# vsergeev/luaradio

Hardware: NVIDIA H100
Metric: WBFM-mono chain Msamples/s (input samples) @N H100; FIR-128 HBM GB/s vs roofline (higher is better)
Workload: dtype f32

## Files before the change

luaradio_b200/csrc/tuner.cu:

```cuda
#include "common.cuh"
#include "blocks.h"

#include <cuda.h>
#include <cudaTypedefs.h>

#include <climits>
#include <cmath>
#include <cstdlib>
#include <cstring>
#include <new>
#include <string>
#include <type_traits>
#include <vector>

namespace lrb {

namespace {

#ifndef LRB_PT_THREADS
#define LRB_PT_THREADS 64
#define LRB_PT_R 8
#define LRB_PT_CTAS 8
#define LRB_PT_PREFETCH 9
#define LRB_PT_BATCH 7
#endif
#ifndef LRB_PT_EXPERIMENT
#define LRB_PT_EXPERIMENT 0
#endif
#ifndef LRB_PT_EARLY_REST
#define LRB_PT_EARLY_REST 0
#endif
constexpr int PT_THREADS = LRB_PT_THREADS;
constexpr int PT_R = LRB_PT_R;
constexpr int PT_TO = PT_THREADS * PT_R;
constexpr int PT_MAXTAPS = 144;
constexpr int PT_BATCH = LRB_PT_BATCH;

constexpr int PT_MAXIT = 48;
struct PolyParams {
    float hr[PT_MAXTAPS];
    float hs[PT_MAXTAPS / 2];
    float2 step[PT_MAXIT];
    uint64_t turns_fix;
    uint64_t g0;
    long long off;
    int M;
    float pole_c;
    float pole_cp[6];
};
constexpr int PT_POLE_WARM = (64 % LRB_PT_R == 0) ? 64 : ((72 % LRB_PT_R == 0) ? 72 : 4 * LRB_PT_R);
static_assert(PT_POLE_WARM % LRB_PT_R == 0 && PT_POLE_WARM % 4 == 0 && PT_POLE_WARM >= 64, "pole warm-up must cover whole threads");

template <int D, int Q>
struct PolyShape {
    static constexpr int RD = PT_R * D;
    static constexpr int T = Q * D + 1;
    static constexpr int SPAN = (PT_TO + Q - 1) * D + 1;
    static constexpr int PAIRS = (SPAN + 1) / 2;
    static constexpr int ITERS = (PAIRS + PT_THREADS - 1) / PT_THREADS;
    static constexpr int LOADED = 2 * ITERS * PT_THREADS;
    __host__ __device__ static constexpr int pad(int e) { return e + 2 * (e / RD); }
    static constexpr int ELEMS = LOADED + 2 * (LOADED / RD) + 2;
    static constexpr size_t SMEM = (size_t)ELEMS * sizeof(float2);
    static constexpr int ROWS = (SPAN + RD - 1) / RD;
    static constexpr int STAGED = ROWS * RD + 2;
    static constexpr size_t SMEM_BULK = (size_t)ROWS * (RD + 2) * sizeof(float2);
    static constexpr int PPS = RD / 2;
    static constexpr int RG = PT_THREADS / PPS;
    static constexpr int RITERS = (ROWS + RG - 1) / RG;
};

__device__ __forceinline__ uint32_t smem_addr(const void* p) { return (uint32_t)__cvta_generic_to_shared(p); }
__device__ __forceinline__ void mbar_init(uint64_t* bar) {
    asm volatile("mbarrier.init.shared::cta.b64 [%0], 1;\n\tfence.mbarrier_init.release.cluster;\n\t"
                 "fence.proxy.async.shared::cta;" :: "r"(smem_addr(bar)) : "memory");
}
__device__ __forceinline__ void mbar_expect_tx(uint64_t* bar, uint32_t bytes) {
    asm volatile("mbarrier.arrive.expect_tx.shared::cta.b64 _, [%0], %1;" :: "r"(smem_addr(bar)), "r"(bytes) : "memory");
}
__device__ __forceinline__ void mbar_wait(uint64_t* bar, uint32_t parity) {
    asm volatile("{\n\t.reg .pred p;\n\tLRB_WAIT_%=:\n\t"
                 "mbarrier.try_wait.parity.shared::cta.b64 p, [%0], %1;\n\t"
                 "@!p bra LRB_WAIT_%=;\n\t}" :: "r"(smem_addr(bar)), "r"(parity) : "memory");
}
__device__ __forceinline__ void fence_proxy_async() { asm volatile("fence.proxy.async.shared::cta;" ::: "memory"); }
__device__ __forceinline__ void tensor_g2s_2d(void* dst, const CUtensorMap* map, int c0, int c1, uint64_t* bar) {
    asm volatile("cp.async.bulk.tensor.2d.shared::cluster.global.tile.mbarrier::complete_tx::bytes [%0], [%1, {%2, %3}], [%4];"
                 :: "r"(smem_addr(dst)), "l"(reinterpret_cast<uint64_t>(map)), "r"(c0), "r"(c1), "r"(smem_addr(bar))
                 : "memory");
}

template <int B, int E, typename F>
__device__ __forceinline__ void static_for(F&& f) {
    if constexpr (B < E) {
        f(std::integral_constant<int, B>{});
        static_for<B + 1, E>(f);
    }
}

constexpr int DISC_OV = 4;
constexpr int DISC_TAIL = 4;
template <bool DISC>
struct TileStride { static constexpr int TS = DISC ? PT_TO - DISC_OV - DISC_TAIL : PT_TO; };

template <int D, int Q, bool ROT, bool DISC, bool EDGE, bool REAL = false, bool POLE = false>
__global__ void __launch_bounds__(PT_THREADS, LRB_PT_CTAS)
polyphase_crcf_kernel(const float2* __restrict__ x, const float2* __restrict__ hist, long long n,
                      void* __restrict__ yv, long long n_out, const __grid_constant__ PolyParams P,
                      const __grid_constant__ CUtensorMap tmap, long long t_lo, long long t_hi,
                      const float2* __restrict__ prev_in, float2* __restrict__ prev_out, float inv_gain) {
    using S = PolyShape<D, Q>;
    static_assert(!(REAL && (ROT || DISC)), "the real-stream variant has no translator / discriminator");
    static_assert(REAL || !POLE, "the fused pole exists in the real-stream variant only");
    constexpr int PW = POLE ? PT_POLE_WARM : 0;
    constexpr int PAY = PT_TO - PW;
    constexpr int TS = REAL ? 2 * PAY : TileStride<DISC>::TS;
    constexpr int NPRE = S::ITERS < LRB_PT_PREFETCH ? S::ITERS : LRB_PT_PREFETCH;
    constexpr int LANE1 = PAY * D;
    const float* __restrict__ xr = reinterpret_cast<const float*>(x);
    const float* __restrict__ histr = reinterpret_cast<const float*>(hist);
    extern __shared__ __align__(128) float2 smem[];
    __shared__ float2 s_edge[PT_THREADS / 32];
    const int tid = threadIdx.x, lane = tid & 31, warp = tid >> 5;
    const int Hm1 = P.M - 1;

    constexpr bool BULK = !EDGE && !REAL && DISC;
    constexpr bool FFA = BULK && LRB_PT_EXPERIMENT != 2;
    __shared__ float2 s_ffa[FFA ? 4 : 1][PT_THREADS / 32];
    __shared__ __align__(8) uint64_t s_bar;
    uint32_t bar_phase = 0;

    float2 A0 = make_float2(1.f, 0.f), A1 = make_float2(1.f, 0.f);
    const int rg = tid / S::PPS, rw = tid - rg * S::PPS;
    constexpr int NE0 = (BULK && ROT) ? S::RITERS : 1;
    float2 E0[NE0];
    float2 W1 = make_float2(1.f, 0.f);
    if constexpr (BULK && ROT) {
        W1 = phasor_from_fix(P.turns_fix);
#pragma unroll
        for (int it = 0; it < NE0; ++it)
            E0[it] = phasor_from_fix(P.turns_fix * (uint64_t)((rg + S::RG * it) * S::RD + 2 * rw));
    } else if constexpr (ROT) {
        A0 = phasor_from_fix(P.turns_fix * (uint64_t)(2 * tid));
        A1 = phasor_from_fix(P.turns_fix * (uint64_t)(2 * tid + 1));
    }
    const bool rot_last = rg < S::RG && rg + S::RG * (S::RITERS - 1) < S::ROWS;
    auto tile_of = [&](long long idx) -> long long { return EDGE ? (idx < t_lo ? idx : t_hi + (idx - t_lo)) : (t_lo + idx); };
    const long long n_work = EDGE ? 0 : (t_hi - t_lo);
    long long widx = blockIdx.x;

    constexpr int TILE_ROWS = TS * D / S::RD;
    static_assert(!BULK || (TS * D) % S::RD == 0, "tiles start on whole rows of the tensor map");
    auto issue_tile = [&](long long idx) {
        if (tid == 0) {
            fence_proxy_async();
            mbar_expect_tx(&s_bar, (uint32_t)S::SMEM_BULK);
            tensor_g2s_2d(smem, &tmap, 0, (int)(idx * TILE_ROWS), &s_bar);
        }
    };
    if constexpr (BULK) {
        if (tid == 0) mbar_init(&s_bar);
        __syncthreads();
        if (widx < n_work) issue_tile(widx);
    }

    auto ld_pair = [&](long long Bt, int k) -> float4 {
        if constexpr (REAL) {
            const float2* pa = reinterpret_cast<const float2*>(xr + Bt) + (tid + k * PT_THREADS);
            const float2 a = __ldcs(pa), b = __ldcs(pa + LANE1 / 2);
            return make_float4(a.x, b.x, a.y, b.y);
        } else {
            return __ldcs(reinterpret_cast<const float4*>(x + Bt) + (tid + k * PT_THREADS));
        }
    };
    float4 pre[NPRE];
    constexpr int REST = (S::ITERS - NPRE) < PT_BATCH ? (S::ITERS - NPRE) : PT_BATCH;
    float4 rest[REST > 0 ? REST : 1];
    if constexpr (!EDGE && !BULK) {
        if (widx < n_work) {
            const long long Bt = P.off + tile_of(widx) * (long long)(TS * D);
#pragma unroll
            for (int k = 0; k < NPRE; ++k) pre[k] = ld_pair(Bt, k);
            if constexpr (LRB_PT_EARLY_REST) {
#pragma unroll
                for (int k = 0; k < REST; ++k) rest[k] = ld_pair(Bt, NPRE + k);
            }
        }
    }

    for (;;) {
        if constexpr (!EDGE) { if (widx >= n_work) break; }
        const long long tile = tile_of(widx);
        const long long B = P.off + tile * (long long)(TS * D);
        const long long m0 = tile * TS - (DISC ? DISC_OV : 0) - PW;

        auto stage_pair = [&](float4 v, int it) {
            const int u = tid + it * PT_THREADS;
            float2 a = make_float2(v.x, v.y), b = make_float2(v.z, v.w);
            if constexpr (ROT) {
                const float2 st = P.step[it];
                a = cmul(a, cmul(A0, st));
                b = cmul(b, cmul(A1, st));
            }
            *reinterpret_cast<float4*>(smem + S::pad(2 * u)) = make_float4(a.x, a.y, b.x, b.y);
        };
        if constexpr (BULK) {
            if (LRB_PT_EXPERIMENT != 1 || widx == blockIdx.x) {
                if (LRB_PT_EXPERIMENT != 3 || widx == blockIdx.x) {
                    mbar_wait(&s_bar, bar_phase);
                    bar_phase ^= 1;
                }
                if (rg < S::RG) {
                    float2* row = smem + rg * (S::RD + 2) + 2 * rw;
#pragma unroll
                    for (int it = 0; it < S::RITERS; ++it) {
                        if (it == S::RITERS - 1 && !rot_last) break;
                        float4* p = reinterpret_cast<float4*>(row + it * S::RG * (S::RD + 2));
                        float4 v = *p;
                        if constexpr (ROT && LRB_PT_EXPERIMENT != 4) {
                            const float2 a = cmul(make_float2(v.x, v.y), E0[it]);
                            const float2 b = cmul(make_float2(v.z, v.w), cmul(E0[it], W1));
                            v = make_float4(a.x, a.y, b.x, b.y);
                        }
                        *p = v;
                    }
                }
            }
        } else if constexpr (!EDGE && LRB_PT_EXPERIMENT == 1) {
            if (widx == blockIdx.x) {
#pragma unroll 1
                for (int it = 0; it < S::ITERS; ++it) stage_pair(ld_pair(B, it), it);
            }
        } else if constexpr (!EDGE) {
            if constexpr (!LRB_PT_EARLY_REST) {
#pragma unroll
                for (int k = 0; k < REST; ++k) rest[k] = ld_pair(B, NPRE + k);
            }
#pragma unroll
            for (int k = 0; k < NPRE; ++k) stage_pair(pre[k], k);
#pragma unroll
            for (int k = 0; k < REST; ++k) stage_pair(rest[k], NPRE + k);
#pragma unroll 1
            for (int it0 = NPRE + REST; it0 < S::ITERS; it0 += PT_BATCH) {
                float4 buf[PT_BATCH];
#pragma unroll
                for (int k = 0; k < PT_BATCH; ++k)
                    if (it0 + k < S::ITERS) buf[k] = ld_pair(B, it0 + k);
#pragma unroll
                for (int k = 0; k < PT_BATCH; ++k)
                    if (it0 + k < S::ITERS) stage_pair(buf[k], it0 + k);
            }
        } else {
#pragma unroll 7
            for (int it = 0; it < S::ITERS; ++it) {
                const long long i0 = B + 2LL * (tid + it * PT_THREADS);
                if constexpr (REAL) {
                    auto g = [&](long long i) -> float {
                        return (i >= 0) ? (i < n ? __ldg(xr + i) : 0.f) : ((Hm1 + i >= 0) ? __ldg(histr + (Hm1 + i)) : 0.f);
                    };
                    stage_pair(make_float4(g(i0), g(i0 + LANE1), g(i0 + 1), g(i0 + 1 + LANE1)), it);
                    continue;
                }
                const float2 a = (i0 >= 0) ? (i0 < n ? __ldg(x + i0) : make_float2(0.f, 0.f))
                                           : ((Hm1 + i0 >= 0) ? __ldg(hist + (Hm1 + i0)) : make_float2(0.f, 0.f));
                const long long i1 = i0 + 1;
                const float2 b = (i1 >= 0) ? (i1 < n ? __ldg(x + i1) : make_float2(0.f, 0.f))
                                           : ((Hm1 + i1 >= 0) ? __ldg(hist + (Hm1 + i1)) : make_float2(0.f, 0.f));
                stage_pair(make_float4(a.x, a.y, b.x, b.y), it);
            }
        }
        __syncthreads();

        if constexpr (!EDGE && !BULK && LRB_PT_EXPERIMENT != 1) {
            const long long nidx = widx + gridDim.x;
            if (nidx < n_work) {
                const long long Bn = P.off + tile_of(nidx) * (long long)(TS * D);
#pragma unroll
                for (int k = 0; k < NPRE; ++k) pre[k] = ld_pair(Bn, k);
            }
        }

        float2 acc[PT_R];
#pragma unroll
        for (int r = 0; r < PT_R; ++r) acc[r] = make_float2(0.f, 0.f);
        const float2* tb = smem + tid * (S::RD + 2);
        auto load_block = [&](auto jc, float2 (&xs)[D]) {
            constexpr int j = decltype(jc)::value;
            constexpr int e0 = j * D;
            if constexpr (j == PT_R + Q - 1) {
                xs[0] = tb[S::pad(e0)];
            } else {
                static_for<0, D>([&](auto pc) {
                    constexpr int pp = decltype(pc)::value;
                    constexpr int e = e0 + pp;
                    if constexpr ((e & 1) && pp >= 1) {
                    } else if constexpr (!(e & 1) && pp + 1 < D) {
                        const float4 v = *reinterpret_cast<const float4*>(tb + S::pad(e));
                        xs[pp] = make_float2(v.x, v.y);
                        xs[pp + 1] = make_float2(v.z, v.w);
                    } else {
                        xs[pp] = tb[S::pad(e)];
                    }
                });
            }
        };
        float2 ffa_a0, ffa_fs, ffa_fb, ffa_sp;
        const float hq = P.hr[Q * D];
        if constexpr (FFA) {
            static_assert(Q % 2 == 0 && PT_R % 2 == 0 && (Q / 2) * D <= PT_MAXTAPS / 2, "fast-FIR split needs even Q and R");
            static_assert(DISC_TAIL >= 1, "the tile's last output has no A_{R/2}");
            constexpr int QH = Q / 2, KP = PT_R / 2;
            float2 fa[KP], fb[KP], fs[KP], uo[D], an;
#pragma unroll
            for (int k = 0; k < KP; ++k) fa[k] = fb[k] = fs[k] = make_float2(0.f, 0.f);
            static_for<0, PT_R + Q>([&](auto jc) {
                constexpr int j = decltype(jc)::value;
                float2 xs[D];
                load_block(jc, xs);
                if constexpr (j == PT_R + Q - 1) {
                } else if constexpr (j % 2 == 0) {
                    constexpr int i = j / 2;
                    static_for<0, KP>([&](auto kc) {
                        constexpr int k = decltype(kc)::value, q = i - k;
                        if constexpr (q >= 0 && q < QH) {
                            static_for<0, D>([&](auto pc) {
                                constexpr int pp = decltype(pc)::value;
                                const float h = P.hr[2 * q * D + pp];
                                fa[k] = ffma2(xs[pp], make_float2(h, h), fa[k]);
                            });
                        }
                    });
                    if constexpr (i >= 1 && i - 1 <= KP - 1 + QH - 1) {
                        float2 v[D];
#pragma unroll
                        for (int pp = 0; pp < D; ++pp) v[pp] = fadd2(uo[pp], xs[pp]);
                        static_for<0, KP>([&](auto kc) {
                            constexpr int k = decltype(kc)::value, q = i - 1 - k;
                            if constexpr (q >= 0 && q < QH) {
                                static_for<0, D>([&](auto pc) {
                                    constexpr int pp = decltype(pc)::value;
                                    const float h = P.hs[q * D + pp];
                                    fs[k] = ffma2(v[pp], make_float2(h, h), fs[k]);
                                });
                            }
                        });
                    }
                } else {
                    constexpr int i = (j - 1) / 2;
                    static_for<0, KP>([&](auto kc) {
                        constexpr int k = decltype(kc)::value, q = i - k;
                        if constexpr (q >= 0 && q < QH) {
                            static_for<0, D>([&](auto pc) {
                                constexpr int pp = decltype(pc)::value;
                                const float h = P.hr[(2 * q + 1) * D + pp];
                                fb[k] = ffma2(xs[pp], make_float2(h, h), fb[k]);
                            });
                        }
                    });
#pragma unroll
                    for (int pp = 0; pp < D; ++pp) uo[pp] = xs[pp];
                }
                if constexpr (j == 2 * QH - 1) {
                    an = make_float2(__shfl_down_sync(0xffffffffu, fa[0].x, 1), __shfl_down_sync(0xffffffffu, fa[0].y, 1));
                }
                if constexpr (j >= Q) {
                    constexpr int r = j - Q, k = r / 2;
                    if constexpr (r % 2 == 0) {
                        acc[r] = ffma2(xs[0], make_float2(hq, hq), fadd2(fa[k], fb[k]));
                    } else if constexpr (k + 1 < KP) {
                        acc[r] = ffma2(xs[0], make_float2(hq, hq), fsub2(fsub2(fs[k], fa[k + 1]), fb[k]));
                    } else {
                        acc[r] = ffma2(xs[0], make_float2(hq, hq), fsub2(fsub2(fs[k], an), fb[k]));
                        ffa_a0 = fa[0]; ffa_fs = fs[k]; ffa_fb = fb[k]; ffa_sp = xs[0];
                    }
                }
            });
        } else {
            static_for<0, (LRB_PT_EXPERIMENT == 2 ? 1 : PT_R + Q)>([&](auto jc) {
                constexpr int j = decltype(jc)::value;
                float2 xs[D];
                load_block(jc, xs);
                static_for<0, PT_R>([&](auto rc) {
                    constexpr int r = decltype(rc)::value;
                    constexpr int qq = j - r;
                    if constexpr (qq >= 0 && qq <= Q) {
                        static_for<0, D>([&](auto pc) {
                            constexpr int pp = decltype(pc)::value;
                            if constexpr (qq * D + pp < S::T) {
                                const float h = P.hr[qq * D + pp];
                                acc[r] = ffma2(xs[pp], make_float2(h, h), acc[r]);
                            }
                        });
                    }
                });
            });
        }
        if constexpr (!EDGE && !BULK && LRB_PT_EARLY_REST) {
            const long long nidx = widx + gridDim.x;
            if (nidx < n_work) {
                const long long Bn = P.off + tile_of(nidx) * (long long)(TS * D);
#pragma unroll
                for (int k = 0; k < REST; ++k) rest[k] = ld_pair(Bn, NPRE + k);
            }
        }
        if constexpr (ROT && !DISC) {
            const float2 Pt = phasor_from_fix(P.turns_fix * (P.g0 + (uint64_t)B));
#pragma unroll
            for (int r = 0; r < PT_R; ++r) acc[r] = cmul(acc[r], Pt);
        }

        const long long mbase = m0 + (long long)tid * PT_R;
        if constexpr (POLE) {
            const float c = P.pole_c;
            if (tile == 0 && tid < PW / PT_R) {
#pragma unroll
                for (int r = 0; r < PT_R; ++r) acc[r].x = 0.f;
                if (tid == PW / PT_R - 1) acc[PT_R - 1].x = __ldg(reinterpret_cast<const float*>(prev_in));
            }
#pragma unroll
            for (int r = 1; r < PT_R; ++r) acc[r] = ffma2(acc[r - 1], make_float2(c, c), acc[r]);
            float2 Bv = acc[PT_R - 1];
#pragma unroll
            for (int k = 0; k < 5; ++k) {
                const float2 o = make_float2(__shfl_up_sync(0xffffffffu, Bv.x, 1 << k), __shfl_up_sync(0xffffffffu, Bv.y, 1 << k));
                if (lane >= (1 << k)) Bv = ffma2(o, make_float2(P.pole_cp[k], P.pole_cp[k]), Bv);
            }
            if (lane == 31) s_edge[warp] = Bv;
            float2 prevB = make_float2(__shfl_up_sync(0xffffffffu, Bv.x, 1), __shfl_up_sync(0xffffffffu, Bv.y, 1));
            if (lane == 0) prevB = make_float2(0.f, 0.f);
            __syncthreads();
            float2 carryW = make_float2(0.f, 0.f);
            for (int w = 0; w < warp; ++w) carryW = ffma2(carryW, make_float2(P.pole_cp[5], P.pole_cp[5]), s_edge[w]);
            float f_lane = 1.f;
#pragma unroll
            for (int k = 0; k < 5; ++k) if (lane & (1 << k)) f_lane *= P.pole_cp[k];
            const float2 excl = ffma2(carryW, make_float2(f_lane, f_lane), prevB);
            float cpow = c;
#pragma unroll
            for (int r = 0; r < PT_R; ++r) { acc[r] = ffma2(excl, make_float2(cpow, cpow), acc[r]); cpow *= c; }
        }
        if constexpr (REAL) {
            float* y = reinterpret_cast<float*>(yv);
#pragma unroll
            for (int half = 0; half < 2; ++half) {
                const long long mb = mbase + half * PAY;
                if (POLE && tid < PW / PT_R) continue;
                float v[PT_R];
#pragma unroll
                for (int r = 0; r < PT_R; ++r) v[r] = half ? acc[r].y : acc[r].x;
                if (mb + PT_R <= n_out && ((reinterpret_cast<uintptr_t>(y + mb) & 15) == 0)) {
#pragma unroll
                    for (int r = 0; r < PT_R; r += 4)
                        __stcs(reinterpret_cast<float4*>(y + mb + r), make_float4(v[r], v[r + 1], v[r + 2], v[r + 3]));
                } else {
#pragma unroll
                    for (int r = 0; r < PT_R; ++r)
                        if (mb + r < n_out) y[mb + r] = v[r];
                }
                if constexpr (POLE) {
                    if (mb <= n_out - 1 && n_out - 1 < mb + PT_R) {
#pragma unroll
                        for (int r = 0; r < PT_R; ++r)
                            if (mb + r == n_out - 1) *reinterpret_cast<float*>(prev_out) = v[r];
                    }
                }
            }
            __syncthreads();
        } else if constexpr (!DISC) {
            float2* y = reinterpret_cast<float2*>(yv);
            if (mbase + PT_R <= n_out && ((reinterpret_cast<uintptr_t>(y + mbase) & 15) == 0)) {
                float4* y4 = reinterpret_cast<float4*>(y + mbase);
#pragma unroll
                for (int r = 0; r < PT_R; r += 2)
                    __stcs(y4 + r / 2, make_float4(acc[r].x, acc[r].y, acc[r + 1].x, acc[r + 1].y));
            } else {
#pragma unroll
                for (int r = 0; r < PT_R; ++r)
                    if (mbase + r < n_out) y[mbase + r] = acc[r];
            }
            __syncthreads();
        } else {
            float* yd = reinterpret_cast<float*>(yv);
            float2 left;
            left.x = __shfl_up_sync(0xffffffffu, acc[PT_R - 1].x, 1);
            left.y = __shfl_up_sync(0xffffffffu, acc[PT_R - 1].y, 1);
            if constexpr (FFA) {
                if (lane == 0) s_ffa[0][warp] = ffa_a0;
                if (lane == 31) { s_ffa[1][warp] = ffa_fs; s_ffa[2][warp] = ffa_fb; s_ffa[3][warp] = ffa_sp; }
            } else {
                if (lane == 31) s_edge[warp] = acc[PT_R - 1];
            }
            __syncthreads();
            if constexpr (BULK && LRB_PT_EXPERIMENT != 1 && LRB_PT_EXPERIMENT != 3) {
                if (widx + gridDim.x < n_work) issue_tile(widx + gridDim.x);
            }
            if constexpr (FFA) {
                auto last_out = [&](int w, float2 a) {
                    return ffma2(s_ffa[3][w], make_float2(hq, hq), fsub2(fsub2(s_ffa[1][w], a), s_ffa[2][w]));
                };
                if (lane == 0 && warp > 0) left = last_out(warp - 1, ffa_a0);
                if (lane == 31 && warp + 1 < PT_THREADS / 32) acc[PT_R - 1] = last_out(warp, s_ffa[0][warp + 1]);
            } else {
                if (lane == 0 && warp > 0) left = s_edge[warp - 1];
            }
            bool zero_prev = false;
            if (EDGE && tid == 0 && tile == 0) {
                const float2 Pt = ROT ? phasor_from_fix(P.turns_fix * (P.g0 + (uint64_t)B)) : make_float2(1.f, 0.f);
                const float2 pv = __ldg(prev_in);
                acc[DISC_OV - 1] = cmul(pv, make_float2(Pt.x, -Pt.y));
                zero_prev = pv.x == 0.f && pv.y == 0.f;
            }
            const int s0 = tid * PT_R;
            float* yt = yd + m0;
            float dout[PT_R];
#pragma unroll
            for (int r = 0; r < PT_R; r += 2) {
                const float2 c0 = acc[r], p0 = (r == 0) ? left : acc[r - 1];
                const float2 c1 = acc[r + 1], p1 = acc[r];
                const float2 t0 = ffma2(c0, make_float2(p0.x, p0.x), fmul2(make_float2(c0.y, -c0.x), make_float2(p0.y, p0.y)));
                const float2 t1 = ffma2(c1, make_float2(p1.x, p1.x), fmul2(make_float2(c1.y, -c1.x), make_float2(p1.y, p1.y)));
                const float2 ang = (!EDGE && LRB_PT_EXPERIMENT == 5) ? make_float2(t0.y, t1.y)
                                                                     : fast_atan2f_x2(make_float2(t0.y, t1.y), make_float2(t0.x, t1.x));
                dout[r] = ang.x * inv_gain;
                dout[r + 1] = ang.y * inv_gain;
            }
            if (EDGE && zero_prev) {
                const float2 Pt = ROT ? phasor_from_fix(P.turns_fix * (P.g0 + (uint64_t)B)) : make_float2(1.f, 0.f);
                const float2 ya = ROT ? cmul(acc[DISC_OV], Pt) : acc[DISC_OV];
                const float pz = 0.f, nz = -0.f;
                const float re = __fsub_rn(__fmul_rn(ya.x, pz), __fmul_rn(ya.y, nz));
                const float im = __fadd_rn(__fmul_rn(ya.x, nz), __fmul_rn(ya.y, pz));
                dout[DISC_OV] = atan2f(im, re) * inv_gain;
            }
            if constexpr (!EDGE) {
                if (((reinterpret_cast<uintptr_t>(yt) + DISC_OV * sizeof(float)) & 15) == 0) {
                    static_assert(DISC_OV == 4 && DISC_TAIL == 4 && PT_R % 4 == 0,
                                  "thread 0 skips exactly its first float4, the last thread exactly its last");
#pragma unroll
                    for (int r = 0; r < PT_R; r += 4)
                        if ((tid > 0 || r >= DISC_OV) && (tid < PT_THREADS - 1 || r < PT_R - DISC_TAIL))
                            *reinterpret_cast<float4*>(yt + s0 + r) = make_float4(dout[r], dout[r + 1], dout[r + 2], dout[r + 3]);
                } else {
#pragma unroll
                    for (int r = 0; r < PT_R; ++r)
                        if (s0 + r >= DISC_OV && s0 + r < PT_TO - DISC_TAIL) yt[s0 + r] = dout[r];
                }
            } else {
                const long long room = n_out - m0;
                const int lim = room < (long long)(PT_TO - DISC_TAIL) ? (int)room : PT_TO - DISC_TAIL;
#pragma unroll
                for (int r = 0; r < PT_R; ++r) {
                    const int sl = s0 + r;
                    if (sl >= DISC_OV && sl < lim) {
                        yt[sl] = dout[r];
                        if ((long long)sl == room - 1) {
                            const float2 Pt = ROT ? phasor_from_fix(P.turns_fix * (P.g0 + (uint64_t)B)) : make_float2(1.f, 0.f);
                            *prev_out = cmul(acc[r], Pt);
                        }
                    }
                }
            }
        }
        if constexpr (EDGE) break;
        widx += gridDim.x;
    }
}

int encode_tile_map(CUtensorMap* map, const float2* base, long long rows, int rd, int box_rows) {
    static const PFN_cuTensorMapEncodeTiled encode = []() -> PFN_cuTensorMapEncodeTiled {
        void* fn = nullptr;
        cudaDriverEntryPointQueryResult q = cudaDriverEntryPointSymbolNotFound;
        if (cudaGetDriverEntryPoint("cuTensorMapEncodeTiled", &fn, cudaEnableDefault, &q) != cudaSuccess ||
            q != cudaDriverEntryPointSuccess)
            return nullptr;
        return reinterpret_cast<PFN_cuTensorMapEncodeTiled>(fn);
    }();
    if (!encode) {
        set_error("tuner: the driver has no cuTensorMapEncodeTiled");
        return -1;
    }
    const cuuint64_t dims[2] = {(cuuint64_t)(2 * (rd + 2)), (cuuint64_t)rows};
    const cuuint64_t strides[1] = {(cuuint64_t)rd * sizeof(float2)};
    const cuuint32_t box[2] = {(cuuint32_t)(2 * (rd + 2)), (cuuint32_t)box_rows};
    const cuuint32_t elem_strides[2] = {1, 1};
    const CUresult r = encode(map, CU_TENSOR_MAP_DATA_TYPE_FLOAT32, 2, const_cast<float2*>(base), dims, strides, box,
                              elem_strides, CU_TENSOR_MAP_INTERLEAVE_NONE, CU_TENSOR_MAP_SWIZZLE_NONE,
                              CU_TENSOR_MAP_L2_PROMOTION_L2_256B, CU_TENSOR_MAP_FLOAT_OOB_FILL_NONE);
    if (r != CUDA_SUCCESS) {
        set_error("tuner: cuTensorMapEncodeTiled failed (CUresult %d)", (int)r);
        return -1;
    }
    return 0;
}

template <int D, int Q, bool ROT, bool DISC, bool REAL = false, bool POLE = false>
int launch_shape(PolyParams P, const float* hr_base, const float2* x, const float2* hist, long long n,
                 void* y, long long first, long long n_out, const float2* prev_in, float2* prev_out, float inv_gain,
                 cudaStream_t s) {
    using S = PolyShape<D, Q>;
    static_assert(S::T <= PT_MAXTAPS, "taps table too small");
    static bool configured_dev[LRB_MAX_DEVICES] = {false};
    static int ctas_dev[LRB_MAX_DEVICES] = {0};
    bool& configured = configured_dev[ctx().device & (LRB_MAX_DEVICES - 1)];
    int& ctas_per_sm = ctas_dev[ctx().device & (LRB_MAX_DEVICES - 1)];
    auto kern_i = polyphase_crcf_kernel<D, Q, ROT, DISC, false, REAL, POLE>;
    auto kern_e = polyphase_crcf_kernel<D, Q, ROT, DISC, true, REAL, POLE>;
    constexpr bool BULK = !REAL && DISC;
    constexpr size_t SMEM_I = BULK ? S::SMEM_BULK : S::SMEM;
    static_assert(!BULK || S::SMEM_BULK >= (size_t)(S::pad(S::SPAN - 1) + 1) * sizeof(float2),
                  "the tensor copy covers every sample a tile reads");
    if (!configured) {
        LRB_CHECK(cudaFuncSetAttribute(kern_i, cudaFuncAttributeMaxDynamicSharedMemorySize, (int)SMEM_I));
        LRB_CHECK(cudaFuncSetAttribute(kern_e, cudaFuncAttributeMaxDynamicSharedMemorySize, (int)S::SMEM));
        LRB_CHECK(cudaOccupancyMaxActiveBlocksPerMultiprocessor(&ctas_per_sm, kern_i, PT_THREADS, SMEM_I));
        if (ctas_per_sm < 1) ctas_per_sm = 1;
        configured = true;
    }
    constexpr int PW = POLE ? PT_POLE_WARM : 0;
    constexpr int PAY = PT_TO - PW;
    constexpr int TS = REAL ? 2 * PAY : TileStride<DISC>::TS;
    long long off = first - (DISC ? (long long)DISC_OV * D : 0) - (long long)PW * D - (long long)(Q * D - 1);
    const int shift = (int)(((off % 2) + 2) % 2);
    off -= shift;
    P.off = off;
    for (int i = 0; i < PT_MAXTAPS; ++i) {
        const int k = i - shift;
        P.hr[i] = (k >= 0 && k < Q * D) ? hr_base[k] : 0.0f;
    }
    for (int q = 0; 2 * q + 1 < Q; ++q)
        for (int p = 0; p < D; ++p) P.hs[q * D + p] = P.hr[2 * q * D + p] + P.hr[(2 * q + 1) * D + p];
    const long long tiles = (n_out + TS - 1) / TS;
    cudaEvent_t lead_event = ctx().lead_samples > 0 ? ctx().lead_event : nullptr;
    const long long lead = lead_event ? ctx().lead_samples : 0;
    const long long step = (long long)TS * D;
    constexpr int TILE_ROWS = TS * D / S::RD;
    long long t_lo = 0, t_hi = 0;
    if ((reinterpret_cast<uintptr_t>(x) & (REAL ? 7 : 15)) == 0) {
        const long long need = lead - off;
        t_lo = need <= 0 ? 0 : (need + step - 1) / step;
        const long long lim = n - (long long)(BULK ? S::STAGED : S::LOADED) - off - (REAL ? (long long)PAY * D : 0);
        t_hi = lim < 0 ? 0 : lim / step + 1;
        if (t_hi > tiles) t_hi = tiles;
        if (DISC) {
            if (t_lo < 1) t_lo = 1;
            if (t_hi > tiles - 1) t_hi = tiles - 1;
        }
        if (t_lo > t_hi) t_lo = t_hi;
        if (BULK && t_hi - t_lo > (INT_MAX - S::ROWS) / TILE_ROWS) t_hi = t_lo + (INT_MAX - S::ROWS) / TILE_ROWS;
    }
    const long long n_int = t_hi - t_lo, n_edge = tiles - n_int;
    CUtensorMap tmap;
    std::memset(&tmap, 0, sizeof(tmap));
    if (BULK && n_int > 0 &&
        encode_tile_map(&tmap, x + off + t_lo * step, (n_int - 1) * TILE_ROWS + S::ROWS, S::RD, S::ROWS) != 0)
        return -1;
    cudaStream_t side = ((n_int > 0 && n_edge > 0) || (lead_event && n_edge > 0)) ? side_fork(s) : s;
    if (n_edge > 0) {
        if (lead_event && side != s) LRB_CHECK(cudaStreamWaitEvent(side, lead_event, 0));
        else if (lead_event) LRB_CHECK(cudaStreamWaitEvent(s, lead_event, 0));
        kern_e<<<(unsigned)n_edge, PT_THREADS, S::SMEM, side>>>(x, hist, n, y, n_out, P, tmap, t_lo, t_hi, prev_in, prev_out, inv_gain);
        count_launch();
    }
    if (n_int > 0) {
        long long grid = (long long)ctx().sm_count * ctas_per_sm - ctx().reserve_ctas;
        if (grid < 1) grid = 1;
        if (grid > n_int) grid = n_int;
        kern_i<<<(unsigned)grid, PT_THREADS, SMEM_I, s>>>(x, hist, n, y, n_out, P, tmap, t_lo, t_hi, prev_in, prev_out, inv_gain);
        count_launch();
    }
    side_join(s, side);
    LRB_CHECK(cudaGetLastError());
    return 1;
}

}

struct PolyTaps {
    int M, D, Q;
    float hr[PT_MAXTAPS];
    uint64_t turns_fix;
    float2 step[PT_MAXIT];
    bool rotates = false;
    bool real_data = false;
};

static int shape_q(int M, int D, bool rotates) {
    if (D == 1 && !rotates) return M <= 16 ? 16 : (M <= 32 ? 32 : 0);
    if (D == 5 && M > 65 && M <= 128) return 26;
    return 0;
}

static int shape_q_real(int M, int D) {
    if (D == 5 && M > 130 && M <= 135) return 27;
    return 0;
}

PolyTaps* polyphase_prepare(const float* taps, int M, int D, double turns_per_sample, bool phasor_table, bool real_data) {
    int Q = real_data ? shape_q_real(M, D) : shape_q(M, D, phasor_table);
    if (!Q) return nullptr;
    PolyTaps* p = new (std::nothrow) PolyTaps();
    if (!p) return nullptr;
    p->M = M; p->D = D; p->Q = Q;
    p->real_data = real_data;
    for (int i = 0; i < PT_MAXTAPS; ++i) {
        int k = Q * D - 1 - i;
        p->hr[i] = (i < Q * D && k < M) ? taps[k] : 0.0f;
    }
    p->turns_fix = turns_to_fix(turns_per_sample);
    p->rotates = phasor_table;
    {
        const double two_pi = 6.283185307179586476925286766559;
        const long double tq = ldexpl((long double)p->turns_fix, -64);
        for (int it = 0; it < PT_MAXIT; ++it) {
            long double a = tq * (long double)(2 * PT_THREADS) * (long double)it;
            a -= floorl(a);
            p->step[it] = make_float2((float)std::cos(two_pi * (double)a), (float)std::sin(two_pi * (double)a));
        }
    }
    return p;
}

void polyphase_release(PolyTaps* p) { delete p; }

#define LRB_SHAPE_FULL(DD, QQ)                                                                                         \
    if (p->D == DD && p->Q == QQ) {                                                                                    \
        static_assert(PolyShape<DD, QQ>::ITERS <= PT_MAXIT, "step table too short");                                   \
        if (disc) return launch_shape<DD, QQ, true, true>(P, p->hr, x, hist, n, y, first, n_out, prev_in, prev_out, inv_gain, s); \
        return rot ? launch_shape<DD, QQ, true, false>(P, p->hr, x, hist, n, y, first, n_out, nullptr, nullptr, 0.f, s)    \
                   : launch_shape<DD, QQ, false, false>(P, p->hr, x, hist, n, y, first, n_out, nullptr, nullptr, 0.f, s);  \
    }
#define LRB_SHAPE_PLAIN(DD, QQ)                                                                                        \
    if (p->D == DD && p->Q == QQ && !rot && !disc) {                                                                   \
        static_assert(PolyShape<DD, QQ>::ITERS <= PT_MAXIT, "step table too short");                                   \
        return launch_shape<DD, QQ, false, false>(P, p->hr, x, hist, n, y, first, n_out, nullptr, nullptr, 0.f, s); \
    }

static int launch_polyphase_any(const PolyTaps* p, const float2* x, const float2* hist, long long n, void* y,
                                long long first, long long n_out, bool rotate, bool disc, uint64_t g0,
                                const float2* prev_in, float2* prev_out, float inv_gain, cudaStream_t s) {
    if (!p) return 0;
    if (n_out <= 0) return 1;
    const bool rot = rotate && p->rotates;
    if (disc && !rot) {
        set_error("tuner: discriminator fusion needs the translator path");
        return -1;
    }
    PolyParams P;
    std::memset(&P, 0, sizeof(P));
    P.turns_fix = p->turns_fix;
    std::memcpy(P.step, p->step, sizeof(P.step));
    P.g0 = g0;
    P.M = p->M;
    if (p->real_data) {
        if (rot || disc) { set_error("polyphase: the real-stream kernel has no translator / discriminator"); return -1; }
        const bool pole = prev_in != nullptr;
        if (pole) {
            const double c = (double)inv_gain;
            P.pole_c = inv_gain;
            double pw = std::pow(c, (double)PT_R);
            for (int k = 0; k < 6; ++k) { P.pole_cp[k] = (float)pw; pw = pw * pw; }
        }
        if (p->D == 5 && p->Q == 27)
            return pole ? launch_shape<5, 27, false, false, true, true>(P, p->hr, x, hist, n, y, first, n_out, prev_in, prev_out, 0.f, s)
                        : launch_shape<5, 27, false, false, true, false>(P, p->hr, x, hist, n, y, first, n_out, nullptr, nullptr, 0.f, s);
        return 0;
    }
    LRB_SHAPE_PLAIN(1, 16) LRB_SHAPE_PLAIN(1, 32)
    LRB_SHAPE_FULL(5, 26)
    return 0;
}

bool polyphase_pole_ok(float c) { return std::pow(std::fabs((double)c), (double)PT_POLE_WARM) <= 1e-8; }

int launch_polyphase_rrrf(const PolyTaps* p, const float* x, const float* hist, long long n, float* y,
                          long long first, long long n_out, cudaStream_t s, float pole_c, const float* z_in, float* z_out) {
    return launch_polyphase_any(p, (const float2*)x, (const float2*)hist, n, y, first, n_out, false, false, 0,
                                (const float2*)z_in, (float2*)z_out, pole_c, s);
}

int launch_polyphase_crcf(const PolyTaps* p, const float2* x, const float2* hist, long long n, float2* y,
                          long long first, long long n_out, bool rotate, uint64_t turns_fix, uint64_t g0,
                          cudaStream_t s) {
    (void)turns_fix;
    return launch_polyphase_any(p, x, hist, n, y, first, n_out, rotate, false, g0, nullptr, nullptr, 0.f, s);
}

struct TunerBlock : Block {
    int M, D;
    std::unique_ptr<PolyTaps> pt;
    DeviceBuffer d_hist[2];
    DeviceBuffer d_prev[2];
    int cur = 0, pcur = 0;
    bool disc = false;
    float gain = 1.f;
    std::string label;

    TunerBlock(std::unique_ptr<PolyTaps>&& p, float disc_gain) : M(p->M), D(p->D), pt(std::move(p)) {
        disc = disc_gain != 0.0f;
        gain = disc_gain;
        in_size = 8;
        out_size = disc ? 4 : 8;
        dev_ptrs = true;
        label = std::string(disc ? "tuner+discrim(" : "tuner(") + std::to_string(M) + ",/" + std::to_string(D) + ")";
        name = label.c_str();
    }
    int init() override {
        return carry(d_hist, (size_t)(M > 1 ? M - 1 : 1) * 8, cur) != 0 || carry(d_prev, 8, pcur) != 0 ? -1 : 0;
    }
    size_t max_output(size_t n) const override { return n / D + 1; }
    uint64_t outputs_before(uint64_t idx) const override { return (idx + D - 1) / D; }
    long long memory_in() const override { return M - 1 + (disc ? D : 0); }
    bool supports_lead_wait() const override { return true; }
    bool state_only_on_side_stream() const override { return true; }
    void rate(unsigned* up, unsigned* down) const override { *up = 1; *down = (unsigned)D; }
    int run(const void* dx, size_t n, void* dy, size_t* n_out, cudaStream_t s) override {
        long long first, no;
        decim_plan(consumed, (unsigned)D, n, &first, &no);
        *n_out = (size_t)no;
        if (n == 0) return 0;
        cudaStream_t side = s;
        if (M > 1) {
            if (n >= SIDE_STREAM_MIN) side = side_fork(s);
            if (launch_hist_update(dx, (long long)n, d_hist[cur].get(), d_hist[cur ^ 1].get(), M - 1, 8, side) != 0) return -1;
        }
        int rc = launch_polyphase_any(pt.get(), (const float2*)dx, d_hist[cur].as<const float2>(), (long long)n, dy, first, no, true,
                                      disc, consumed, d_prev[pcur].as<const float2>(), d_prev[pcur ^ 1].as<float2>(),
                                      disc ? 1.0f / gain : 0.f, s);
        side_join(s, side);
        if (rc <= 0) { if (rc == 0) set_error("tuner: unsupported shape"); return -1; }
        if (disc && no > 0) pcur ^= 1;
        if (M > 1) cur ^= 1;
        consumed += n;
        return 0;
    }
};

std::unique_ptr<Block> make_tuner(double turns_per_sample, const float* taps, int ntaps, int decim, float disc_gain) {
    std::unique_ptr<PolyTaps> p(polyphase_prepare(taps, ntaps, decim, turns_per_sample, true));
    if (!p) return nullptr;
    return make_block<TunerBlock>(std::move(p), disc_gain);
}

}
```

Measured before the change: 226,600.

## Run bulk tuner tiles as multi-group CTAs sharing a TMA slot ring

The bulk (TMA) interior kernel now launches one CTA per SM that holds several independent thread groups. The groups share a ring of shared-memory slots that are refilled ahead of use, so each tile load has more lookahead than the old single buffer per small CTA. Groups synchronise with named barriers and release/acquire flags on per-slot issue counters. The change adds register caps and a hard failure if more than one CTA fits per SM, and it risks spin-wait overhead and lower occupancy flexibility.

```diff
diff --git a/luaradio_b200/csrc/tuner.cu b/luaradio_b200/csrc/tuner.cu
--- a/luaradio_b200/csrc/tuner.cu
+++ b/luaradio_b200/csrc/tuner.cu
@@ -30,6 +30,10 @@
 #ifndef LRB_PT_EARLY_REST
 #define LRB_PT_EARLY_REST 0
 #endif
+#ifndef LRB_PT_RING_GROUPS
+#define LRB_PT_RING_GROUPS 6
+#define LRB_PT_RING_SLOTS 10
+#endif
 constexpr int PT_THREADS = LRB_PT_THREADS;
 constexpr int PT_R = LRB_PT_R;
 constexpr int PT_TO = PT_THREADS * PT_R;
@@ -37,6 +41,13 @@
 constexpr int PT_BATCH = LRB_PT_BATCH;
 
 constexpr int PT_MAXIT = 48;
+constexpr int PT_RING_G = LRB_PT_RING_GROUPS;
+constexpr int PT_RING_S = LRB_PT_RING_SLOTS;
+static_assert(PT_RING_G >= 1 && PT_RING_G <= 15 && PT_RING_S > PT_RING_G, "ring: 1..15 groups and more slots than groups");
+constexpr int PT_RING_WARPS = (PT_RING_G * PT_THREADS / 32 + 3) / 4 * 4;
+constexpr int PT_RING_REGS = (65536 / (PT_RING_WARPS * 32) / 8 * 8) < 255 ? (65536 / (PT_RING_WARPS * 32) / 8 * 8) : 255;
+template <bool EDGE, bool REAL, bool DISC>
+__host__ __device__ constexpr bool pt_ring() { return !EDGE && !REAL && DISC; }
 struct PolyParams {
     float hr[PT_MAXTAPS];
     float hs[PT_MAXTAPS / 2];
@@ -65,6 +76,8 @@
     static constexpr int ROWS = (SPAN + RD - 1) / RD;
     static constexpr int STAGED = ROWS * RD + 2;
     static constexpr size_t SMEM_BULK = (size_t)ROWS * (RD + 2) * sizeof(float2);
+    static constexpr int SLOT = (int)((SMEM_BULK + 127) / 128 * 128 / sizeof(float2));
+    static constexpr size_t SMEM_RING = (size_t)PT_RING_S * SLOT * sizeof(float2);
     static constexpr int PPS = RD / 2;
     static constexpr int RG = PT_THREADS / PPS;
     static constexpr int RITERS = (ROWS + RG - 1) / RG;
@@ -84,6 +97,15 @@
                  "@!p bra LRB_WAIT_%=;\n\t}" :: "r"(smem_addr(bar)), "r"(parity) : "memory");
 }
 __device__ __forceinline__ void fence_proxy_async() { asm volatile("fence.proxy.async.shared::cta;" ::: "memory"); }
+__device__ __forceinline__ void st_release_cta(int* p, int v) {
+    asm volatile("st.release.cta.shared::cta.b32 [%0], %1;" :: "r"(smem_addr(p)), "r"(v) : "memory");
+}
+__device__ __forceinline__ int ld_acquire_cta(const int* p) {
+    int v;
+    asm volatile("ld.acquire.cta.shared::cta.b32 %0, [%1];" : "=r"(v) : "r"(smem_addr(p)) : "memory");
+    return v;
+}
+__device__ __forceinline__ void named_sync(int id, int n) { asm volatile("bar.sync %0, %1;" :: "r"(id), "r"(n) : "memory"); }
 __device__ __forceinline__ void tensor_g2s_2d(void* dst, const CUtensorMap* map, int c0, int c1, uint64_t* bar) {
     asm volatile("cp.async.bulk.tensor.2d.shared::cluster.global.tile.mbarrier::complete_tx::bytes [%0], [%1, {%2, %3}], [%4];"
                  :: "r"(smem_addr(dst)), "l"(reinterpret_cast<uint64_t>(map)), "r"(c0), "r"(c1), "r"(smem_addr(bar))
@@ -104,7 +126,9 @@
 struct TileStride { static constexpr int TS = DISC ? PT_TO - DISC_OV - DISC_TAIL : PT_TO; };
 
 template <int D, int Q, bool ROT, bool DISC, bool EDGE, bool REAL = false, bool POLE = false>
-__global__ void __launch_bounds__(PT_THREADS, LRB_PT_CTAS)
+__global__ void __launch_bounds__(pt_ring<EDGE, REAL, DISC>() ? PT_RING_G * PT_THREADS : PT_THREADS,
+                                  pt_ring<EDGE, REAL, DISC>() ? 0 : LRB_PT_CTAS)
+__maxnreg__((pt_ring<EDGE, REAL, DISC>() ? PT_RING_REGS : 65536 / (PT_THREADS * LRB_PT_CTAS)))
 polyphase_crcf_kernel(const float2* __restrict__ x, const float2* __restrict__ hist, long long n,
                       void* __restrict__ yv, long long n_out, const __grid_constant__ PolyParams P,
                       const __grid_constant__ CUtensorMap tmap, long long t_lo, long long t_hi,
@@ -120,15 +144,24 @@
     const float* __restrict__ xr = reinterpret_cast<const float*>(x);
     const float* __restrict__ histr = reinterpret_cast<const float*>(hist);
     extern __shared__ __align__(128) float2 smem[];
-    __shared__ float2 s_edge[PT_THREADS / 32];
-    const int tid = threadIdx.x, lane = tid & 31, warp = tid >> 5;
+    constexpr bool BULK = pt_ring<EDGE, REAL, DISC>();
+    constexpr int NG = BULK ? PT_RING_G : 1;
+    constexpr int WPG = PT_THREADS / 32;
+    __shared__ float2 s_edge[NG * WPG];
+    const int grp = BULK ? (int)threadIdx.x / PT_THREADS : 0;
+    const int tid = BULK ? (int)threadIdx.x - grp * PT_THREADS : (int)threadIdx.x, lane = tid & 31, warp = tid >> 5;
+    const int gw = grp * WPG + warp;
     const int Hm1 = P.M - 1;
 
-    constexpr bool BULK = !EDGE && !REAL && DISC;
     constexpr bool FFA = BULK && LRB_PT_EXPERIMENT != 2;
-    __shared__ float2 s_ffa[FFA ? 4 : 1][PT_THREADS / 32];
-    __shared__ __align__(8) uint64_t s_bar;
-    uint32_t bar_phase = 0;
+    __shared__ float2 s_ffa[FFA ? 4 : 1][NG * WPG];
+    constexpr int NS = BULK ? PT_RING_S : 1;
+    __shared__ __align__(8) uint64_t s_bar[NS];
+    __shared__ int s_issued[NS];
+    auto group_sync = [&]() {
+        if constexpr (BULK) named_sync(1 + grp, PT_THREADS);
+        else __syncthreads();
+    };
 
     float2 A0 = make_float2(1.f, 0.f), A1 = make_float2(1.f, 0.f);
     const int rg = tid / S::PPS, rw = tid - rg * S::PPS;
@@ -147,21 +180,31 @@
     const bool rot_last = rg < S::RG && rg + S::RG * (S::RITERS - 1) < S::ROWS;
     auto tile_of = [&](long long idx) -> long long { return EDGE ? (idx < t_lo ? idx : t_hi + (idx - t_lo)) : (t_lo + idx); };
     const long long n_work = EDGE ? 0 : (t_hi - t_lo);
-    long long widx = blockIdx.x;
+    int kt = grp;
+    long long widx = blockIdx.x + (long long)grp * gridDim.x;
+    const long long wstep = (long long)NG * gridDim.x;
+    const int n_cta = BULK ? (int)((n_work - blockIdx.x + gridDim.x - 1) / gridDim.x) : 0;
 
     constexpr int TILE_ROWS = TS * D / S::RD;
     static_assert(!BULK || (TS * D) % S::RD == 0, "tiles start on whole rows of the tensor map");
-    auto issue_tile = [&](long long idx) {
-        if (tid == 0) {
-            fence_proxy_async();
-            mbar_expect_tx(&s_bar, (uint32_t)S::SMEM_BULK);
-            tensor_g2s_2d(smem, &tmap, 0, (int)(idx * TILE_ROWS), &s_bar);
-        }
+    auto issue_tile = [&](int k, long long idx) {
+        const int slot = k % NS;
+        fence_proxy_async();
+        mbar_expect_tx(&s_bar[slot], (uint32_t)S::SMEM_BULK);
+        tensor_g2s_2d(smem + slot * S::SLOT, &tmap, 0, (int)(idx * TILE_ROWS), &s_bar[slot]);
+        st_release_cta(&s_issued[slot], k);
     };
+    constexpr bool ONE_COPY = LRB_PT_EXPERIMENT == 1 || LRB_PT_EXPERIMENT == 3;
     if constexpr (BULK) {
-        if (tid == 0) mbar_init(&s_bar);
+        if (threadIdx.x < NS) {
+            mbar_init(&s_bar[threadIdx.x]);
+            s_issued[threadIdx.x] = -1;
+        }
         __syncthreads();
-        if (widx < n_work) issue_tile(widx);
+        if (threadIdx.x == 0) {
+            const int first = n_cta < (ONE_COPY ? NG : NS) ? n_cta : (ONE_COPY ? NG : NS);
+            for (int k = 0; k < first; ++k) issue_tile(k, blockIdx.x + (long long)k * gridDim.x);
+        }
     }
 
     auto ld_pair = [&](long long Bt, int k) -> float4 {
@@ -204,14 +247,16 @@
             }
             *reinterpret_cast<float4*>(smem + S::pad(2 * u)) = make_float4(a.x, a.y, b.x, b.y);
         };
+        float2* const tbuf = BULK ? smem + (kt % NS) * S::SLOT : smem;
         if constexpr (BULK) {
-            if (LRB_PT_EXPERIMENT != 1 || widx == blockIdx.x) {
-                if (LRB_PT_EXPERIMENT != 3 || widx == blockIdx.x) {
-                    mbar_wait(&s_bar, bar_phase);
-                    bar_phase ^= 1;
+            if (LRB_PT_EXPERIMENT != 1 || kt < NG) {
+                if (LRB_PT_EXPERIMENT != 3 || kt < NG) {
+                    const int slot = kt % NS;
+                    while (ld_acquire_cta(&s_issued[slot]) != kt) __nanosleep(64);
+                    mbar_wait(&s_bar[slot], (uint32_t)(kt / NS) & 1u);
                 }
                 if (rg < S::RG) {
-                    float2* row = smem + rg * (S::RD + 2) + 2 * rw;
+                    float2* row = tbuf + rg * (S::RD + 2) + 2 * rw;
 #pragma unroll
                     for (int it = 0; it < S::RITERS; ++it) {
                         if (it == S::RITERS - 1 && !rot_last) break;
@@ -269,7 +314,7 @@
                 stage_pair(make_float4(a.x, a.y, b.x, b.y), it);
             }
         }
-        __syncthreads();
+        group_sync();
 
         if constexpr (!EDGE && !BULK && LRB_PT_EXPERIMENT != 1) {
             const long long nidx = widx + gridDim.x;
@@ -283,7 +328,7 @@
         float2 acc[PT_R];
 #pragma unroll
         for (int r = 0; r < PT_R; ++r) acc[r] = make_float2(0.f, 0.f);
-        const float2* tb = smem + tid * (S::RD + 2);
+        const float2* tb = tbuf + tid * (S::RD + 2);
         auto load_block = [&](auto jc, float2 (&xs)[D]) {
             constexpr int j = decltype(jc)::value;
             constexpr int e0 = j * D;
@@ -485,23 +530,23 @@
             left.x = __shfl_up_sync(0xffffffffu, acc[PT_R - 1].x, 1);
             left.y = __shfl_up_sync(0xffffffffu, acc[PT_R - 1].y, 1);
             if constexpr (FFA) {
-                if (lane == 0) s_ffa[0][warp] = ffa_a0;
-                if (lane == 31) { s_ffa[1][warp] = ffa_fs; s_ffa[2][warp] = ffa_fb; s_ffa[3][warp] = ffa_sp; }
+                if (lane == 0) s_ffa[0][gw] = ffa_a0;
+                if (lane == 31) { s_ffa[1][gw] = ffa_fs; s_ffa[2][gw] = ffa_fb; s_ffa[3][gw] = ffa_sp; }
             } else {
-                if (lane == 31) s_edge[warp] = acc[PT_R - 1];
-            }
-            __syncthreads();
-            if constexpr (BULK && LRB_PT_EXPERIMENT != 1 && LRB_PT_EXPERIMENT != 3) {
-                if (widx + gridDim.x < n_work) issue_tile(widx + gridDim.x);
+                if (lane == 31) s_edge[gw] = acc[PT_R - 1];
+            }
+            group_sync();
+            if constexpr (BULK && !ONE_COPY) {
+                if (tid == 0 && kt + NS < n_cta) issue_tile(kt + NS, widx + (long long)NS * gridDim.x);
             }
             if constexpr (FFA) {
                 auto last_out = [&](int w, float2 a) {
                     return ffma2(s_ffa[3][w], make_float2(hq, hq), fsub2(fsub2(s_ffa[1][w], a), s_ffa[2][w]));
                 };
-                if (lane == 0 && warp > 0) left = last_out(warp - 1, ffa_a0);
-                if (lane == 31 && warp + 1 < PT_THREADS / 32) acc[PT_R - 1] = last_out(warp, s_ffa[0][warp + 1]);
+                if (lane == 0 && warp > 0) left = last_out(gw - 1, ffa_a0);
+                if (lane == 31 && warp + 1 < WPG) acc[PT_R - 1] = last_out(gw, s_ffa[0][gw + 1]);
             } else {
-                if (lane == 0 && warp > 0) left = s_edge[warp - 1];
+                if (lane == 0 && warp > 0) left = s_edge[gw - 1];
             }
             bool zero_prev = false;
             if (EDGE && tid == 0 && tile == 0) {
@@ -562,7 +607,8 @@
             }
         }
         if constexpr (EDGE) break;
-        widx += gridDim.x;
+        widx += wstep;
+        kt += NG;
     }
 }
 
@@ -605,16 +651,22 @@
     int& ctas_per_sm = ctas_dev[ctx().device & (LRB_MAX_DEVICES - 1)];
     auto kern_i = polyphase_crcf_kernel<D, Q, ROT, DISC, false, REAL, POLE>;
     auto kern_e = polyphase_crcf_kernel<D, Q, ROT, DISC, true, REAL, POLE>;
-    constexpr bool BULK = !REAL && DISC;
-    constexpr size_t SMEM_I = BULK ? S::SMEM_BULK : S::SMEM;
+    constexpr bool BULK = pt_ring<false, REAL, DISC>();
+    constexpr size_t SMEM_I = BULK ? S::SMEM_RING : S::SMEM;
+    constexpr int THREADS_I = BULK ? PT_RING_G * PT_THREADS : PT_THREADS;
     static_assert(!BULK || S::SMEM_BULK >= (size_t)(S::pad(S::SPAN - 1) + 1) * sizeof(float2),
                   "the tensor copy covers every sample a tile reads");
     if (!configured) {
         LRB_CHECK(cudaFuncSetAttribute(kern_i, cudaFuncAttributeMaxDynamicSharedMemorySize, (int)SMEM_I));
         LRB_CHECK(cudaFuncSetAttribute(kern_e, cudaFuncAttributeMaxDynamicSharedMemorySize, (int)S::SMEM));
-        LRB_CHECK(cudaOccupancyMaxActiveBlocksPerMultiprocessor(&ctas_per_sm, kern_i, PT_THREADS, SMEM_I));
-        if (ctas_per_sm < 1) ctas_per_sm = 1;
+        LRB_CHECK(cudaOccupancyMaxActiveBlocksPerMultiprocessor(&ctas_per_sm, kern_i, THREADS_I, SMEM_I));
+        if (!BULK && ctas_per_sm < 1) ctas_per_sm = 1;
         configured = true;
+    }
+    if (BULK && ctas_per_sm != 1) {
+        set_error("tuner: the ring kernel fits %d CTAs per SM instead of 1 (%d threads, %zu B of shared memory)",
+                  ctas_per_sm, THREADS_I, SMEM_I);
+        return -1;
     }
     constexpr int PW = POLE ? PT_POLE_WARM : 0;
     constexpr int PAY = PT_TO - PW;
@@ -662,10 +714,11 @@
         count_launch();
     }
     if (n_int > 0) {
-        long long grid = (long long)ctx().sm_count * ctas_per_sm - ctx().reserve_ctas;
+        long long grid = BULK ? (long long)ctx().sm_count - (ctx().reserve_ctas + PT_RING_G - 1) / PT_RING_G
+                              : (long long)ctx().sm_count * ctas_per_sm - ctx().reserve_ctas;
         if (grid < 1) grid = 1;
         if (grid > n_int) grid = n_int;
-        kern_i<<<(unsigned)grid, PT_THREADS, SMEM_I, s>>>(x, hist, n, y, n_out, P, tmap, t_lo, t_hi, prev_in, prev_out, inv_gain);
+        kern_i<<<(unsigned)grid, THREADS_I, SMEM_I, s>>>(x, hist, n, y, n_out, P, tmap, t_lo, t_hi, prev_in, prev_out, inv_gain);
         count_launch();
     }
     side_join(s, side);
```

New measurement: 230,700, median of 6. 1.8% higher.
